# TJUMMG/OCPG

Hardware: AMD Instinct MI355X
Metric: clips/sec fwd+bwd (5x384x640, R101) (higher is better)
Workload: dtype bf16

## Files before the change

include/ocpg_hip.h:

```cpp
#ifndef OCPG_HIP_H
#define OCPG_HIP_H
#include <stdint.h>

#ifdef __cplusplus
extern "C" {
#endif

int ocpg_msda_fwd_f32(const float* value, const int64_t* shapes, const int64_t* level_start,
                      const float* loc, const float* attn,
                      int N, int S, int M, int D, int L, int Lq, int P,
                      float* out, const int64_t* shapes_host, void* stream);
int ocpg_msda_fwd_f64(const double* value, const int64_t* shapes, const int64_t* level_start,
                      const double* loc, const double* attn,
                      int N, int S, int M, int D, int L, int Lq, int P,
                      double* out, void* stream);

int ocpg_msda_bwd_f32(const float* value, const int64_t* shapes, const int64_t* level_start,
                      const float* loc, const float* attn, const float* grad_out,
                      int N, int S, int M, int D, int L, int Lq, int P,
                      float* grad_value, float* grad_loc, float* grad_attn,
                      const int64_t* shapes_host, void* stream);
int ocpg_msda_bwd_value_f32(const float* loc, const float* attn, const float* grad_out,
                            int N, int S, int M, int D, int L, int Lq, int P,
                            float* grad_value, const int64_t* shapes_host, void* stream);
// ... 31 lines not shown
int ocpg_msda_fwd_h16(const void* value, const int64_t* shapes, const int64_t* level_start,
                      const float* loc, const float* attn,
                      int N, int S, int M, int D, int L, int Lq, int P,
                      void* out, const int64_t* shapes_host, int dtype, void* stream);
int ocpg_msda_bwd_h16(const void* value, const int64_t* shapes, const int64_t* level_start,
                      const float* loc, const float* attn, const void* grad_out,
                      int N, int S, int M, int D, int L, int Lq, int P,
                      float* grad_value, float* grad_loc, float* grad_attn,
                      const int64_t* shapes_host, int* sel_state, int dtype, void* stream);
int ocpg_msda_bwd_value_h16(const float* loc, const float* attn, const void* grad_out,
                            int N, int S, int M, int D, int L, int Lq, int P,
                            float* grad_value, const int64_t* shapes_host, int* sel_state, int dtype, void* stream);
int ocpg_msda_bwd_locattn_h16(const void* value, const int64_t* shapes, const int64_t* level_start,
                              const float* loc, const float* attn, const void* grad_out,
                              int N, int S, int M, int D, int L, int Lq, int P,
                              float* grad_loc, float* grad_attn, int dtype, void* stream);
int ocpg_msda_fused_fwd_h16(const void* value, const int64_t* shapes, const int64_t* level_start,
                            const float* qproj, const float* ref,
                            int N, int S, int M, int D, int L, int Lq, int P,
                            void* out, float* loc_out, float* attn_out, int dtype, void* stream);
int ocpg_msda_fused_bwd_qproj_h16(const void* value, const int64_t* shapes, const int64_t* level_start,
                                  const float* loc, const float* attn, const void* grad_out,
                                  int N, int S, int M, int D, int L, int Lq, int P,
                                  float* grad_qproj, int dtype, void* stream);

int ocpg_bn_act_fwd(const void* x, const float* scale, const float* shift, const void* skip, void* y,
                    long long n_outer, int C, long long inner, int relu, int dtype, void* stream);
int ocpg_bn_act_bwd(const void* gy, const void* y, const float* scale, void* gx, void* gskip,
                    long long n_outer, int C, long long inner, int relu, int dtype, void* stream);

int ocpg_gemm_dgrad_bn_tile(long long M, int N, int K);
int ocpg_gemm_dgrad_bn(const void* a, const void* w, const void* c, const void* mask, const float* scale, void* out, void* out_skip,
                       long long M, int N, int K, int dtype, int tile, void* stream);

int ocpg_win_attn_fwd(const void* qkv, const float* biasT, const int* region, float scale, int BW, int NW, int N, int H,
                      int head_dim, void* out, float* lse, int dtype, void* stream);
int ocpg_win_attn_bwd(const void* qkv, const float* bias, const float* biasT, const int* region, float scale, int BW, int NW,
                      int N, int H, int head_dim, const void* out, const void* dout, const float* lse, void* dqkv, float* Dbuf,
                      float* dbiasT, int dtype, void* stream);

int ocpg_win_attn_bwd_mfma(const void* qkv, const float* bias, const float* biasT, const int* region, float scale, int BW, int NW, int N,
                           int H, int head_dim, const void* out, const void* dout, const float* lse, void* dqkv, float* Dbuf, void* dS,
                           int dtype, void* stream);

int ocpg_win_attn_dtable_supported(int N, int head_dim, int dtype, int T);
int ocpg_win_attn_bwd_mfma_dtable(const void* qkv, const float* bias, const float* biasT, const int* region, float scale, int BW, int NW,
                                  int N, int H, int head_dim, const void* out, const void* dout, const float* lse, void* dqkv, float* Dbuf,
                                  const int* tok_code, int code_off, int T, float* partials, float* dtable, int dtype, void* stream);

int ocpg_dynmask_fwd_f32(const float* feats, const float* params, const float* refpix, int BT, int Q, int C, int H, int W,
                         int stride, float* out, float* pre1, void* stream);

int ocpg_dynmask_bwd_pre_f32(const float* dout, const float* pre1, const float* params, int BT, int Q, int C, int H, int W,
                             int stride, float* dpre, float* part, float* w0d, void* stream);
int ocpg_dynmask_bwd_fin_f32(const float* part, const float* params, const float* refpix, const float* dw0, int BT, int Q, int C,
                             int H, int W, float* dparams, float* dref, void* stream);

int ocpg_im2col3x3_nhwc(const void* x, int N, int H, int W, int C, int stride, int dil, void* cols, int dtype, void* stream);
int ocpg_col2im3x3_nhwc(const void* dcols, int N, int H, int W, int C, int stride, int dil, void* dx, int dtype, void* stream);

int ocpg_conv3x3_mfma_fwd(const void* x, const void* w, const float* scale, const float* bias, int relu, int N, int H, int W,
                          int Cin, int Cout, int stride, void* y, void* stream);
int ocpg_conv3x3_mfma_fwd_cols(const void* x, const void* w, const float* scale, const float* bias, int relu, int N, int H, int W, int Cin,
                               int Cout, int stride, void* y, void* cols, void* stream);
int ocpg_conv3x3_mfma_dgrad(const void* dy, const void* wT, int N, int H, int W, int Cin, int Cout, int stride, void* dx,
                            void* stream);
int ocpg_conv3x3_mfma_dgrad_masked(const void* dy, const void* wT, const void* mask_y, const float* scale, int N, int H, int W, int Cin,
                                   int Cout, int stride, void* dx, void* stream);
int ocpg_conv3x3_mfma_dgrad_w(const void* dy, const void* w, const void* mask_y, const float* scale, int N, int H, int W, int Cin, int Cout,
                              int stride, void* dx, void* stream);
int ocpg_conv3x3_mfma_body_splits(long long M, int ncols, int kchannels);
int ocpg_conv3x3_mfma_fwd_bn_splitk(const void* x, const void* w, const float* scale, const float* shift, int relu, int N, int H, int W, int Cin,
                                    int Cout, int stride, int splits, float* part, void* y, void* stream);
int ocpg_conv3x3_mfma_dgrad_w_splitk(const void* dy, const void* w, const void* mask_y, const float* scale, int N, int H, int W, int Cin,
                                     int Cout, int stride, int splits, float* part, void* dx, void* stream);
int ocpg_conv3x3_mfma_wgrad_splits(int N, int H, int W, int Cin, int Cout, int stride);
int ocpg_conv3x3_mfma_wgrad(const void* gz, const void* x, int N, int H, int W, int Cin, int Cout, int stride, void* part, void* stream);
int ocpg_conv3x3_mfma_fwd_cols_h16(const void* x, const void* w, const float* scale, const float* bias, int relu, int N, int H, int W, int Cin,
                                   int Cout, int stride, void* y, void* cols, int dtype, void* stream);
int ocpg_conv3x3_mfma_dgrad_w_h16(const void* dy, const void* w, const void* mask_y, const float* scale, int N, int H, int W, int Cin, int Cout,
                                  int stride, void* dx, int dtype, void* stream);
int ocpg_conv3x3_mfma_wgrad_h16(const void* gz, const void* x, int N, int H, int W, int Cin, int Cout, int stride, void* part, int dtype,
                                void* stream);
int ocpg_conv3x3_mfma_dgrad_w_s2(const void* dy, const void* w, const void* mask_y, const float* scale, int N, int H, int W, int Cin, int Cout,
                                 int stride, void* dx, void* stream);
int ocpg_conv3x3_mfma_dgrad_w_s2_h16(const void* dy, const void* w, const void* mask_y, const float* scale, int N, int H, int W, int Cin, int Cout,
                                     int stride, void* dx, int dtype, void* stream);

int ocpg_conv3x3_mfma_splits(int N, int H, int W, int Cin, int Cout, int stride);
int ocpg_conv3x3_mfma_fwd_splitk(const void* x, const void* w, const float* bias, int N, int H, int W, int Cin, int Cout, int stride,
                                 int splits, float* part, void* y, int out_dt, void* cols, void* stream);
int ocpg_conv3x3_mfma_fwd_splitk_h16(const void* x, const void* w, const float* bias, int N, int H, int W, int Cin, int Cout, int stride,
                                     int splits, float* part, void* y, int out_dt, void* cols, int dtype, void* stream);

int ocpg_gemm(const void* A, const void* B, void* C, const void* bias, int dtype, int out_dtype, int transA, int transB,
              long long M, long long N, long long K, long long lda, long long ldb, long long ldc, long long batch,
              long long strideA, long long strideB, long long strideC, float alpha, float beta, void* stream);
long long ocpg_gemm_plans(void);
long long ocpg_gemm_tuned(long long* changed);
long long ocpg_gemm_tune_rejected(void);
void ocpg_gemm_set_tuning(int on);
long long ocpg_gemm_export_picks(long long* buf, long long cap_pairs);
int ocpg_gemm_import_picks(const long long* buf, long long n_pairs);
int ocpg_gemm_bn_act(const void* A, const void* W, void* D, const float* scale, const float* shift, const void* skip, int relu, int dtype,
                     long long M, long long N, long long K, void* stream);

int ocpg_levelset_fwd_f32(const float* x, const float* feats, const float* box, int Lr, int N, int C, int CF, int h, int w, float* sums,
                          float* coef, float* loss, void* stream);
int ocpg_levelset_bwd_f32(const float* x, const float* feats, const float* box, const float* coef, const float* gloss, int Lr, int N,
                          int C, int CF, int h, int w, float* gx, float* gfeat, void* stream);
int ocpg_proj_fwd_f32(const float* x, const float* tcmax, const float* trmax, const float* tcmean, const float* trmean, int Lr, int B,
                      int T, int H, int W, float* colstat, float* rowstat, float* IU, float* loss, void* stream);
int ocpg_proj_bwd_f32(const float* x, const float* tcmax, const float* trmax, const float* tcmean, const float* trmean,
                      const float* colstat, const float* rowstat, const float* IU, const float* gloss, int Lr, int B, int T, int H, int W,
                      float* Gc, float* Gr, float* gx, void* stream);

int ocpg_matcher_cost_f32(const float* logits, const float* boxes, const float* masks, long long sl, long long sb, long long st,
                          long long sq, const float* gt, const float* tboxes, const float* valid, const long long* labels, int Lr,
                          int B, int T, int Q, int K, int h, int w, float wc, float wb, float wg, float wm, float wd, float* sums,
                          float* cost, int* bad, void* stream);

int ocpg_dropout_add_ln_fwd(const void* x, const float* res, const float* gamma, const float* beta, long long R, int C, float eps, float p,
                            unsigned long long seed, unsigned long long offset, const unsigned long long* rng_base, int x_dtype, float* y,
                            float* mean, float* rstd, void* stream);
int ocpg_dropout_add_ln_bwd(const float* gy, const void* x, const float* res, const float* gamma, const float* mean, const float* rstd,
                            long long R, int C, float p, unsigned long long seed, unsigned long long offset, const unsigned long long* rng_base,
                            int x_dtype, void* gx, float* gres, float* dgb_part, void* stream);
long long ocpg_dropout_add_ln_bwd_slots(long long R);
int ocpg_bias_relu_dropout_fwd(const void* a, const void* bias, long long R, int C, float p, unsigned long long seed,
                               unsigned long long offset, const unsigned long long* rng_base, int dtype, void* h, void* stream);
int ocpg_bias_relu_dropout_bwd(const void* gh, const void* h, long long R, int C, float p, int dtype, void* ga, float* dbias_part,
                               void* stream);
long long ocpg_bias_relu_dropout_bwd_slots(long long R, int C, int dtype);

int ocpg_multi_cast(const long long* srcs, const long long* dsts, const long long* numels, const long long* chunk_prefix, int n,
                    long long total_chunks, int src_dtype, int dst_dtype, void* stream);
int ocpg_multi_cast_sum(const long long* srcs, const long long* dsts, const long long* numels, const long long* chunk_prefix,
                        const long long* splits, const long long* strides, int n, long long total_chunks, int src_dtype, int dst_dtype,
                        void* stream);
long long ocpg_colsum_blocks(long long R);
int ocpg_colsum_partials(const void* x, long long R, int C, int dtype, float* part, void* stream);

int ocpg_grad_norm_clip(const long long* grads, const long long* numels, const long long* chunk_prefix, int n, long long total_chunks,
                        float max_norm, float* partials, float* norm_and_coef, void* stream);
int ocpg_adamw_step(const long long* params, const long long* grads, const long long* exp_avg, const long long* exp_avg_sq,
                    const long long* numels, const long long* chunk_prefix, const float* lr, const float* weight_decay, int n,
                    long long total_chunks, const float* norm_and_coef, double beta1, double beta2, double eps, long long step, void* stream);
int ocpg_grad_norm_clip_amp(const long long* grads, const long long* numels, const long long* chunk_prefix, int n, long long total_chunks,
                            float max_norm, float* partials, const float* grad_scale, const float* found_inf, double beta1, double beta2,
                            float* amp_state, void* stream);
int ocpg_adamw_step_amp(const long long* params, const long long* grads, const long long* exp_avg, const long long* exp_avg_sq,
                        const long long* numels, const long long* chunk_prefix, const float* lr, const float* weight_decay, int n,
                        long long total_chunks, const float* amp_state, double beta1, double beta2, double eps, void* stream);

int ocpg_det_loss_fwd_f32(const float* logits, const float* boxes, const long long* src, const float* valid, const long long* labels,
                          const float* tboxes, const float* num_boxes, float alpha, int Lr, int B, int T, int Q, int K, float* loss, int* bad,
                          void* stream);
int ocpg_det_loss_bwd_f32(const float* logits, const float* boxes, const long long* src, const float* valid, const long long* labels,
                          const float* tboxes, const float* num_boxes, const float* gloss, float alpha, int Lr, int B, int T, int Q, int K,
                          float* glogits, float* gboxes, void* stream);

int ocpg_spectral_gate_fwd(const void* X, const float* coef, const float* high, int N, int C, int hw, float* out, void* stream);
int ocpg_spectral_c2p(const void* X, const float* coef, const float* high, int N, int C, int hw, void* pair, int dtype, void* stream);
int ocpg_spectral_p2c(const void* pair, const void* Xs, const float* coef, const float* high, int N, int C, int hw, void* out, float* part,
                      int dtype, void* stream);
int ocpg_spectral_gate_bwd(const float* gout, const void* X, const float* coef, const float* high, int N, int C, int hw, void* dX, float* part,
// ... 81 lines not shown
```

ocpg_amd/_lib.py:

```python
import ctypes
import os

import torch

_HERE = os.path.dirname(os.path.abspath(__file__))
LIB_PATH = os.environ.get("OCPG_HIP_LIB") or os.path.join(_HERE, "lib", "libocpg_hip.so")
_lib = None

_i64p = ctypes.c_void_p
_vp = ctypes.c_void_p
_int = ctypes.c_int

SIGNATURES = {
    "ocpg_msda_fwd_f32": [_vp, _i64p, _i64p, _vp, _vp] + [_int] * 7 + [_vp, _vp, _vp],
    "ocpg_msda_fwd_f64": [_vp, _i64p, _i64p, _vp, _vp] + [_int] * 7 + [_vp, _vp],
    "ocpg_msda_bwd_f32": [_vp, _i64p, _i64p, _vp, _vp, _vp] + [_int] * 7 + [_vp, _vp, _vp, _vp, _vp],
    "ocpg_msda_bwd_value_f32": [_vp, _vp, _vp] + [_int] * 7 + [_vp, _vp, _vp],
    "ocpg_msda_fused_fwd_f32": [_vp, _i64p, _i64p, _vp, _vp] + [_int] * 7 + [_vp, _vp, _vp, _vp],
    "ocpg_msda_fused_bwd_qproj_f32": [_vp, _i64p, _i64p, _vp, _vp, _vp] + [_int] * 7 + [_vp, _vp],
    "ocpg_msda_bwd_value_sel_f32": [_vp, _vp, _vp] + [_int] * 7 + [_vp, _vp, _vp, _vp],
    "ocpg_msda_bwd_locattn_f32": [_vp, _i64p, _i64p, _vp, _vp, _vp] + [_int] * 7 + [_vp, _vp, _vp],
    "ocpg_msda_bwd_f64": [_vp, _i64p, _i64p, _vp, _vp, _vp] + [_int] * 7 + [_vp, _vp, _vp, _vp],
    "ocpg_msda_sf_fwd_f32": [_vp, _vp, _vp, _vp, _i64p, _i64p, _vp, _vp] + [_int] * 7 + [_vp, _vp, _vp, _vp],
    "ocpg_msda_sf_bwd_f32": [_vp, _vp, _vp, _vp, _i64p, _i64p, _vp, _vp, _vp] + [_int] * 7 + [_vp, _vp, _vp, _vp],
    "ocpg_msda_sf_bwd_params_f32": [_vp, _vp, _vp] + [_int] * 4 + [_vp, _vp, _vp],
    "ocpg_msda_fwd_h16": [_vp, _i64p, _i64p, _vp, _vp] + [_int] * 7 + [_vp, _vp, _int, _vp],
    "ocpg_msda_bwd_h16": [_vp, _i64p, _i64p, _vp, _vp, _vp] + [_int] * 7 + [_vp, _vp, _vp, _vp, _vp, _int, _vp],
    "ocpg_msda_bwd_value_h16": [_vp, _vp, _vp] + [_int] * 7 + [_vp, _vp, _vp, _int, _vp],
    "ocpg_msda_bwd_locattn_h16": [_vp, _i64p, _i64p, _vp, _vp, _vp] + [_int] * 7 + [_vp, _vp, _int, _vp],
    "ocpg_msda_fused_fwd_h16": [_vp, _i64p, _i64p, _vp, _vp] + [_int] * 7 + [_vp, _vp, _vp, _int, _vp],
    "ocpg_msda_fused_bwd_qproj_h16": [_vp, _i64p, _i64p, _vp, _vp, _vp] + [_int] * 7 + [_vp, _int, _vp],
    "ocpg_bn_act_fwd": [_vp, _vp, _vp, _vp, _vp, ctypes.c_longlong, _int, ctypes.c_longlong, _int, _int, _vp],
    "ocpg_bn_act_bwd": [_vp, _vp, _vp, _vp, _vp, ctypes.c_longlong, _int, ctypes.c_longlong, _int, _int, _vp],
    "ocpg_gemm_dgrad_bn_tile": [ctypes.c_longlong, _int, _int],
    "ocpg_gemm_dgrad_bn": [_vp] * 7 + [ctypes.c_longlong, _int, _int, _int, _int, _vp],
    "ocpg_dynmask_fwd_f32": [_vp, _vp, _vp] + [_int] * 6 + [_vp, _vp, _vp],
    "ocpg_dynmask_bwd_pre_f32": [_vp, _vp, _vp] + [_int] * 6 + [_vp, _vp, _vp, _vp],
    "ocpg_dynmask_bwd_fin_f32": [_vp, _vp, _vp, _vp] + [_int] * 5 + [_vp, _vp, _vp],
    "ocpg_conv3x3_mfma_fwd": [_vp, _vp, _vp, _vp] + [_int] * 7 + [_vp, _vp],
    "ocpg_conv3x3_mfma_fwd_cols": [_vp, _vp, _vp, _vp] + [_int] * 7 + [_vp, _vp, _vp],
    "ocpg_conv3x3_mfma_dgrad": [_vp, _vp] + [_int] * 6 + [_vp, _vp],
    "ocpg_conv3x3_mfma_dgrad_masked": [_vp, _vp, _vp, _vp] + [_int] * 6 + [_vp, _vp],
    "ocpg_conv3x3_mfma_dgrad_w": [_vp, _vp, _vp, _vp] + [_int] * 6 + [_vp, _vp],
    "ocpg_conv3x3_mfma_splits": [_int] * 6,
    "ocpg_conv3x3_mfma_wgrad_splits": [_int] * 6,
    "ocpg_conv3x3_mfma_body_splits": [ctypes.c_longlong, _int, _int],
    "ocpg_conv3x3_mfma_fwd_bn_splitk": [_vp, _vp, _vp, _vp] + [_int] * 8 + [_vp, _vp, _vp],
    "ocpg_conv3x3_mfma_dgrad_w_splitk": [_vp, _vp, _vp, _vp] + [_int] * 7 + [_vp, _vp, _vp],
    "ocpg_conv3x3_mfma_wgrad": [_vp, _vp] + [_int] * 6 + [_vp, _vp],
    "ocpg_conv3x3_mfma_fwd_cols_h16": [_vp, _vp, _vp, _vp] + [_int] * 7 + [_vp, _vp, _int, _vp],
    "ocpg_conv3x3_mfma_dgrad_w_h16": [_vp, _vp, _vp, _vp] + [_int] * 6 + [_vp, _int, _vp],
    "ocpg_conv3x3_mfma_wgrad_h16": [_vp, _vp] + [_int] * 6 + [_vp, _int, _vp],
    "ocpg_conv3x3_mfma_dgrad_w_s2": [_vp, _vp, _vp, _vp] + [_int] * 6 + [_vp, _vp],
    "ocpg_conv3x3_mfma_dgrad_w_s2_h16": [_vp, _vp, _vp, _vp] + [_int] * 6 + [_vp, _int, _vp],
    "ocpg_conv3x3_mfma_fwd_splitk": [_vp, _vp, _vp] + [_int] * 7 + [_vp, _vp, _int, _vp, _vp],
    "ocpg_conv3x3_mfma_fwd_splitk_h16": [_vp, _vp, _vp] + [_int] * 7 + [_vp, _vp, _int, _vp, _int, _vp],
    "ocpg_gemm": [_vp, _vp, _vp, _vp] + [_int] * 4 + [ctypes.c_longlong] * 10 + [ctypes.c_float, ctypes.c_float, _vp],
    "ocpg_gemm_plans": [],
    "ocpg_gemm_tuned": [_vp],
    "ocpg_gemm_tune_rejected": [],
    "ocpg_gemm_set_tuning": [_int],
    "ocpg_gemm_export_picks": [_vp, ctypes.c_longlong],
    "ocpg_gemm_import_picks": [_vp, ctypes.c_longlong],
    "ocpg_window_means3x3_fwd": [_vp, ctypes.c_longlong, _int, _int, _int, _vp, _vp],
    "ocpg_window_means3x3_bwd": [_vp, ctypes.c_longlong, _int, _int, _vp, _vp],
    "ocpg_window_sums3x3_cl_bands": [_int],
    "ocpg_window_sums3x3_cl": [_vp, _int, _int, _int, _int, _int, _vp, _vp],
    "ocpg_window_means3x3_bwd_cl": [_vp, _int, _int, _int, _int, _vp, _vp, _vp],
    "ocpg_mso_conv3x3": [_vp, _int, _int, _vp, _int, _vp, _vp, _int, _vp, _int, _vp, _vp, _int] + [_int] * 6 + [_vp],
    "ocpg_mso_wgrad_rows": [_int] * 4,
    "ocpg_mso_wgrad": [_vp, _int, _int, _vp, _vp, _vp] + [_int] * 8 + [_vp],
    "ocpg_bilinear_nhwc_fwd": [_vp] + [_int] * 6 + [_vp, _vp],
    "ocpg_bilinear_nhwc_bwd": [_vp] + [_int] * 6 + [_vp, _vp],
    "ocpg_small_linear_fwd": [_vp, _int, _vp, _vp, _int, _int, _int, _int, _vp, _vp],
    "ocpg_small_linear_bwd": [_vp, _int, _vp, _int, _vp, _vp, _int, _int, _int, _vp, _vp, _vp, _vp],
    "ocpg_small_linear_fwd_h16": [_vp, _int, _vp, _vp, _int, _int, _int, _int, _vp, _int, _vp],
    "ocpg_small_linear_bwd_h16": [_vp, _int, _vp, _int, _vp, _vp, _int, _int, _int, _vp, _vp, _vp, _int, _vp],
    "ocpg_small_linear_f32_fwd": [_vp, _vp, _vp, _int, _int, _int, _vp, _vp],
    "ocpg_small_linear_f32_bwd": [_vp, _vp, _vp, _int, _int, _int, _vp, _vp, _vp, _vp],
    "ocpg_layernorm_blocks": [ctypes.c_longlong],
    "ocpg_groupnorm_cl_work": [ctypes.c_longlong, _int, _int, _int],
    "ocpg_groupnorm_cl_fwd": [_vp, _int, _vp, _vp, ctypes.c_longlong, _int, _int, _int, ctypes.c_float, _vp, _vp, _vp, _vp, _vp],
    "ocpg_groupnorm_cl_bwd": [_vp, _vp, _int, _vp, _vp, _vp, ctypes.c_longlong, _int, _int, _int, _vp, _vp, _vp, _vp],
    "ocpg_groupnorm_cl2cl_fwd": [_vp, _int, _vp, _vp, ctypes.c_longlong, _int, _int, _int, ctypes.c_float, _vp, _vp, _vp, _vp, _vp],
    "ocpg_groupnorm_cl2cl_bwd": [_vp, _vp, _int, _vp, _vp, _vp, ctypes.c_longlong, _int, _int, _int, _vp, _vp, _vp, _vp],
    "ocpg_layernorm_fwd": [_vp, _int, _vp, _vp, ctypes.c_longlong, _int, ctypes.c_float, _vp, _int, _vp, _vp, _vp],
    "ocpg_layernorm_bwd": [_vp, _int, _vp, _int, _vp, _vp, _vp, ctypes.c_longlong, _int, _vp, _int, _vp, _vp, _vp],
    "ocpg_gather_rows_bwd": [_vp, _vp, _vp, _int, _int, _vp, _vp],
    "ocpg_relpos_bias_fwd": [_vp, _vp, _int, ctypes.c_longlong, _int, _vp, _vp, _vp],
    "ocpg_relpos_bias_bwd": [_vp, _vp, _vp, _int, _int, _int, _int, _vp, _vp],
    "ocpg_gather_rows_pad": [_vp, _vp] + [ctypes.c_longlong] * 4 + [_vp, _vp],
    "ocpg_graph_replace_memsets": [_vp, _vp],
    "ocpg_graph_stats": [_vp, _vp],
    "ocpg_graph_memcpy_nodes": [_vp, _vp, _int],
    "ocpg_gemm_bn_act": [_vp] * 6 + [_int, _int] + [ctypes.c_longlong] * 3 + [_vp],
    "ocpg_levelset_fwd_f32": [_vp] * 3 + [_int] * 6 + [_vp] * 4,
    "ocpg_levelset_bwd_f32": [_vp] * 5 + [_int] * 6 + [_vp] * 3,
    "ocpg_proj_fwd_f32": [_vp] * 5 + [_int] * 5 + [_vp] * 5,
    "ocpg_proj_bwd_f32": [_vp] * 9 + [_int] * 5 + [_vp] * 4,
    "ocpg_matcher_cost_f32": [_vp] * 3 + [ctypes.c_longlong] * 4 + [_vp] * 4 + [_int] * 7 + [ctypes.c_float] * 5 + [_vp] * 4,
    "ocpg_dropout_add_ln_fwd": [_vp] * 4 + [ctypes.c_longlong, _int, ctypes.c_float, ctypes.c_float, ctypes.c_ulonglong, ctypes.c_ulonglong, _vp, _int]
                               + [_vp] * 4,
    "ocpg_dropout_add_ln_bwd": [_vp] * 6 + [ctypes.c_longlong, _int, ctypes.c_float, ctypes.c_ulonglong, ctypes.c_ulonglong, _vp, _int] + [_vp] * 4,
    "ocpg_dropout_add_ln_bwd_slots": [ctypes.c_longlong],
    "ocpg_bias_relu_dropout_fwd": [_vp, _vp, ctypes.c_longlong, _int, ctypes.c_float, ctypes.c_ulonglong, ctypes.c_ulonglong, _vp, _int, _vp, _vp],
    "ocpg_bias_relu_dropout_bwd": [_vp, _vp, ctypes.c_longlong, _int, ctypes.c_float, _int, _vp, _vp, _vp],
    "ocpg_bias_relu_dropout_bwd_slots": [ctypes.c_longlong, _int, _int],
    "ocpg_multi_cast": [_vp] * 4 + [_int, ctypes.c_longlong, _int, _int, _vp],
    "ocpg_multi_cast_sum": [_vp] * 6 + [_int, ctypes.c_longlong, _int, _int, _vp],
    "ocpg_colsum_blocks": [ctypes.c_longlong],
    "ocpg_grad_norm_clip": [_vp] * 3 + [_int, ctypes.c_longlong, ctypes.c_float, _vp, _vp, _vp],
    "ocpg_adamw_step": [_vp] * 8 + [_int, ctypes.c_longlong, _vp, ctypes.c_double, ctypes.c_double, ctypes.c_double, ctypes.c_longlong, _vp],
    "ocpg_grad_norm_clip_amp": [_vp] * 3 + [_int, ctypes.c_longlong, ctypes.c_float, _vp, _vp, _vp, ctypes.c_double, ctypes.c_double, _vp, _vp],
    "ocpg_adamw_step_amp": [_vp] * 8 + [_int, ctypes.c_longlong, _vp, ctypes.c_double, ctypes.c_double, ctypes.c_double, _vp],
    "ocpg_lfm_dft_supported": [_int, _int],
    "ocpg_lfm_dft_split": [_int],
    "ocpg_lfm_spectrum_fwd": [_vp, _vp, _vp] + [_int] * 4 + [_vp, _vp, ctypes.c_float, _vp, _vp, _int, _vp],
    "ocpg_lfm_spectrum_inv": [_vp, _int, _vp, _vp, _vp, _vp] + [_int] * 4 + [_vp, _vp, ctypes.c_float, _vp, _vp, _vp, _vp],
    "ocpg_colsum_partials": [_vp, ctypes.c_longlong, _int, _int, _vp, _vp],
    "ocpg_det_loss_fwd_f32": [_vp] * 7 + [ctypes.c_float] + [_int] * 5 + [_vp] * 3,
    "ocpg_det_loss_bwd_f32": [_vp] * 8 + [ctypes.c_float] + [_int] * 5 + [_vp] * 3,
    "ocpg_spectral_gate_fwd": [_vp] * 3 + [_int] * 3 + [_vp, _vp],
    "ocpg_spectral_gate_bwd": [_vp] * 4 + [_int] * 3 + [_vp, _vp, _vp],
    "ocpg_spectral_c2p": [_vp] * 3 + [_int] * 3 + [_vp, _int, _vp],
    "ocpg_spectral_p2c": [_vp] * 4 + [_int] * 3 + [_vp, _vp, _int, _vp],
    "ocpg_masked_ce_fwd_f32": [_vp] * 3 + [_int, ctypes.c_longlong, _vp, _vp],
    "ocpg_masked_ce_bwd_f32": [_vp] * 4 + [_int, ctypes.c_longlong, _vp, _vp],
    "ocpg_im2col3x3_nhwc": [_vp] + [_int] * 6 + [_vp, _int, _vp],
    "ocpg_col2im3x3_nhwc": [_vp] + [_int] * 6 + [_vp, _int, _vp],
    "ocpg_attn_smallk_fwd": [_vp, ctypes.c_longlong, _vp, ctypes.c_longlong, _vp, ctypes.c_longlong, _vp, ctypes.c_float] + [_int] * 5
                            + [ctypes.c_float, ctypes.c_ulonglong, ctypes.c_ulonglong, _vp, _vp, ctypes.c_longlong, _vp, _int, _vp],
    "ocpg_attn_smallk_bwd": [_vp, ctypes.c_longlong, _vp, ctypes.c_longlong, _vp, ctypes.c_longlong, _vp, _vp, ctypes.c_longlong, _vp,
                             ctypes.c_float] + [_int] * 5 + [ctypes.c_float, ctypes.c_ulonglong, ctypes.c_ulonglong, _vp, _vp, ctypes.c_longlong,
                                                             _vp, _vp, _int, _vp],
    "ocpg_win_attn_fwd": [_vp, _vp, _vp, ctypes.c_float] + [_int] * 5 + [_vp, _vp, _int, _vp],
    "ocpg_win_attn_bwd": [_vp, _vp, _vp, _vp, ctypes.c_float] + [_int] * 5 + [_vp] * 6 + [_int, _vp],
    "ocpg_win_attn_bwd_mfma": [_vp, _vp, _vp, _vp, ctypes.c_float] + [_int] * 5 + [_vp] * 6 + [_int, _vp],
    "ocpg_win_attn_dtable_supported": [_int] * 4,
    "ocpg_win_attn_bwd_mfma_dtable": [_vp, _vp, _vp, _vp, ctypes.c_float] + [_int] * 5 + [_vp] * 6 + [_int, _int, _vp, _vp, _int, _vp],
}


_TIMING = {"on": False, "events": []}
_UNTIMED = ("ocpg_win_attn_dtable_supported", "ocpg_conv3x3_mfma_body_splits", "ocpg_gemm_dgrad_bn_tile", "ocpg_conv3x3_mfma_wgrad_splits", "ocpg_window_sums3x3_cl_bands", "ocpg_lfm_dft_supported", "ocpg_lfm_dft_split", "ocpg_conv3x3_mfma_splits", "ocpg_gemm_set_tuning", "ocpg_gemm_export_picks", "ocpg_gemm_import_picks", "ocpg_colsum_blocks", "ocpg_mso_wgrad_rows", "ocpg_gemm_plans", "ocpg_gemm_tuned", "ocpg_gemm_tune_rejected", "ocpg_bias_relu_dropout_bwd_slots", "ocpg_dropout_add_ln_bwd_slots", "ocpg_groupnorm_cl_work")


def enable_kernel_timing(on=True):
    _TIMING["on"] = on
    _TIMING["events"] = []


def collect_kernel_timing(work=None):
    torch.cuda.synchronize()
    out = {}
    for name, args, e0, e1 in _TIMING["events"]:
        d = out.setdefault(name, {"ms": 0.0, "n": 0, "work": 0.0, "modelled": 0})
        d["ms"] += e0.elapsed_time(e1)
        d["n"] += 1
        w = work(name, args) if work is not None else None
        if isinstance(w, tuple):
            d["work_lowp"] = d.get("work_lowp", 0.0) + (w[0] if w[1] else 0.0)
            w = w[0]
        if w is not None:
            d["work"] += w
            d["modelled"] += 1
    _TIMING["events"] = []
    _TIMING["on"] = False
    return out


CENSUS = {"on": False, "calls": {}}
CENSUS_ALSO = {"ocpg_conv3x3_mfma_dgrad_w_s2": "ocpg_conv3x3_mfma_dgrad_w", "ocpg_conv3x3_mfma_dgrad_w_s2_h16": "ocpg_conv3x3_mfma_dgrad_w_h16"}


def census(on=True):
    CENSUS["on"] = on
    if on:
        CENSUS["calls"] = {}
    return CENSUS["calls"]


class _Lib:

    def __init__(self, cdll):
        self._cdll = cdll

    def __getattr__(self, name):
        fn = getattr(self._cdll, name)
        if name not in SIGNATURES or name in _UNTIMED:
            setattr(self, name, fn)
            return fn
        timed = not name.startswith("ocpg_msda_")

        def call(*a):
            if CENSUS["on"]:
                rc = fn(*a)
                if rc == 0:
                    for k in (name, CENSUS_ALSO.get(name)):
                        if k is not None:
                            CENSUS["calls"][k] = CENSUS["calls"].get(k, 0) + 1
                return rc
            if not (timed and _TIMING["on"]):
                return fn(*a)
            e0, e1 = torch.cuda.Event(enable_timing=True), torch.cuda.Event(enable_timing=True)
            e0.record()
            rc = fn(*a)
            e1.record()
            _TIMING["events"].append((name, tuple(getattr(x, "value", x) for x in a), e0, e1))
            return rc
        setattr(self, name, call)
        return call


def lib():
    global _lib
    if _lib is None:
        if not os.path.exists(LIB_PATH):
            raise RuntimeError(
                f"{LIB_PATH} not found: build it with `python -m ocpg_amd.csrc.build` "
                "(hipcc --offload-arch=gfx950). The HIP extension is mandatory; there is no CPU/PyTorch fallback.")
        L = ctypes.CDLL(LIB_PATH)
        for name, argtypes in SIGNATURES.items():
            fn = getattr(L, name)
            fn.argtypes = argtypes
            fn.restype = ctypes.c_int
        L.ocpg_hip_version.restype = ctypes.c_char_p
        L.ocpg_gemm_plans.restype = ctypes.c_longlong
# ... 29 lines not shown
```

ocpg_amd/csrc/conv3x3_wgrad.hip:

```cpp
#include <hip/hip_bf16.h>
#include <hip/hip_fp16.h>
#include <hip/hip_runtime.h>
#include <stdint.h>

#include <cstdlib>

#include "../../include/ocpg_hip.h"
#include "h16_elem.h"

namespace {

typedef ocpg_h16::h16x8 bf16x8;
typedef short s4 __attribute__((ext_vector_type(4)));
typedef ocpg_h16::f32x16 f32x16;
using ocpg_h16::Bf16;
using ocpg_h16::Fp16;

constexpr int NT = 256, TM = 64, TN = 64, LROW = 72;

__device__ __forceinline__ bf16x8 tr_frag(const short* tile, int r0, int pitch, int c0, int lane) {
  const int li = lane & 15, grp = lane >> 4, fh = lane >> 5;
  const short* p = tile + (r0 + (8 * fh + (li >> 2)) * pitch) * LROW + c0 + 16 * (grp & 1) + 4 * (li & 3);
  const s4 lo = __builtin_amdgcn_ds_read_tr16_b64_v4i16((__attribute__((address_space(3))) s4*)p);
  const s4 hi = __builtin_amdgcn_ds_read_tr16_b64_v4i16((__attribute__((address_space(3))) s4*)(p + 4 * pitch * LROW));
  bf16x8 r;
  r[0] = lo[0]; r[1] = lo[1]; r[2] = lo[2]; r[3] = lo[3]; r[4] = hi[0]; r[5] = hi[1]; r[6] = hi[2]; r[7] = hi[3];
  return r;
}

__device__ __forceinline__ uint4 keep(uint4 v, bool yes) { return make_uint4(yes ? v.x : 0u, yes ? v.y : 0u, yes ? v.z : 0u, yes ? v.w : 0u); }

struct WG {
  int N, H, W, Ho, Wo, Cin, Cout, stride, seg, xw, rows_per_split;
};

#define WGRAD_KERNEL conv3x3_wgrad
#define WGRAD_ELEM Bf16
#include "conv3x3_wgrad_kernel.h"
#undef WGRAD_KERNEL
#undef WGRAD_ELEM
#define WGRAD_KERNEL conv3x3_wgrad_f16
#define WGRAD_ELEM Fp16
#include "conv3x3_wgrad_kernel.h"
#undef WGRAD_KERNEL
#undef WGRAD_ELEM

inline int seg_of(int stride) { return stride == 1 ? 64 : 32; }

}

extern "C" {

int ocpg_conv3x3_mfma_wgrad_splits(int N, int H, int W, int Cin, int Cout, int stride) {
  if (N <= 0 || H <= 0 || W <= 0 || Cin <= 0 || Cout <= 0 || (stride != 1 && stride != 2)) return 0;
  const long long rows = (long long)N * ((H - 1) / stride + 1);
  const long long tiles = (long long)((Cout + TM - 1) / TM) * ((Cin + TN - 1) / TN);
  static const int target = [] { const char* e = std::getenv("OCPG_WGRAD_WGS"); return e && *e ? std::atoi(e) : 256; }();
  long long s = (target + tiles - 1) / tiles;
  if (s > rows) s = rows;
  if (s < 1) s = 1;
  const long long rps = (rows + s - 1) / s;
  return (int)((rows + rps - 1) / rps);
}

int ocpg_conv3x3_mfma_wgrad_h16(const void* gz, const void* x, int N, int H, int W, int Cin, int Cout, int stride, void* part, int dtype,
                                void* stream) {
  if (dtype != 1 && dtype != 2) return -1010;
  if (N < 0 || H <= 0 || W <= 0 || Cin <= 0 || Cout <= 0) return -1003;
  if ((stride != 1 && stride != 2) || Cin % 8 != 0 || Cout % 8 != 0) return -2000;
  if (N == 0) return 0;
  if (!gz) return -1001;
  if (!x) return -1002;
  if (!part) return -1009;
  WG g;
  g.N = N; g.H = H; g.W = W; g.Ho = (H - 1) / stride + 1; g.Wo = (W - 1) / stride + 1; g.Cin = Cin; g.Cout = Cout; g.stride = stride;
  g.seg = seg_of(stride);
  g.xw = (g.seg - 1) * stride + 3;
  const int splits = ocpg_conv3x3_mfma_wgrad_splits(N, H, W, Cin, Cout, stride);
  const long long rows = (long long)N * g.Ho;
  g.rows_per_split = (int)((rows + splits - 1) / splits);
  const dim3 grid((unsigned)((Cout + TM - 1) / TM), (unsigned)((Cin + TN - 1) / TN), (unsigned)splits);
  if (dtype == 2) {
    if (stride == 1) conv3x3_wgrad_f16<1, 64><<<grid, NT, 0, (hipStream_t)stream>>>((const __half*)gz, (const __half*)x, g, (__half*)part);
    else conv3x3_wgrad_f16<2, 32><<<grid, NT, 0, (hipStream_t)stream>>>((const __half*)gz, (const __half*)x, g, (__half*)part);
  } else if (stride == 1) {
    conv3x3_wgrad<1, 64><<<grid, NT, 0, (hipStream_t)stream>>>((const __hip_bfloat16*)gz, (const __hip_bfloat16*)x, g, (__hip_bfloat16*)part);
  } else {
    conv3x3_wgrad<2, 32><<<grid, NT, 0, (hipStream_t)stream>>>((const __hip_bfloat16*)gz, (const __hip_bfloat16*)x, g, (__hip_bfloat16*)part);
  }
  const hipError_t e = hipGetLastError();
  return e == hipSuccess ? 0 : -(int)e;
}

int ocpg_conv3x3_mfma_wgrad(const void* gz, const void* x, int N, int H, int W, int Cin, int Cout, int stride, void* part, void* stream) {
  return ocpg_conv3x3_mfma_wgrad_h16(gz, x, N, H, W, Cin, Cout, stride, part, 1, stream);
}

}
```

ocpg_amd/csrc/conv3x3_wgrad_kernel.h:

```cpp
template <int S, int SEG>
#ifdef WG_ONE_SET
__global__ __launch_bounds__(NT) __attribute__((amdgpu_waves_per_eu(2, 2))) void WGRAD_KERNEL(
#else
__global__ __launch_bounds__(NT) __attribute__((amdgpu_waves_per_eu(1, 1))) void WGRAD_KERNEL(
#endif
    const WGRAD_ELEM::T* __restrict__ gz, const WGRAD_ELEM::T* __restrict__ x, WG g,
                                                    WGRAD_ELEM::T* __restrict__ part) {
  using E = WGRAD_ELEM;
  using T = E::T;
  constexpr int XW = (SEG - 1) * S + 3;
  constexpr int GL = SEG * 8 / NT;
  constexpr int XL = (3 * XW * 8 + NT - 1) / NT;
  __shared__ __attribute__((aligned(16))) short Gs[SEG * LROW];
  __shared__ __attribute__((aligned(16))) short Xs[3 * XW * LROW];
  const int tid = threadIdx.x, lane = tid & 63, wave = tid >> 6, wm = wave & 1, wn = wave >> 1;
  const int co0 = blockIdx.x * TM, ci0 = blockIdx.y * TN;
  const long long rows = (long long)g.N * g.Ho;
  const long long r_lo = (long long)blockIdx.z * g.rows_per_split, r_hi = min(rows, r_lo + g.rows_per_split);
  const int nseg = (g.Wo + SEG - 1) / SEG;
  const int nchunks = (int)(r_hi > r_lo ? r_hi - r_lo : 0) * nseg;
  f32x16 acc[9];
#pragma unroll
  for (int t = 0; t < 9; ++t)
#pragma unroll
    for (int r = 0; r < 16; ++r) acc[t][r] = 0.f;
  struct Regs { uint4 rg[GL], rx[XL]; unsigned zg, zx; };
  Regs RA, RB;
  const long long r0c = min(r_lo, rows - 1);
  int fn = (int)(r0c / g.Ho), fy = (int)(r0c - (long long)fn * g.Ho), fs = 0;
  auto fetch = [&](Regs& R) __attribute__((always_inline)) {
    uint4 (&rg)[GL] = R.rg; uint4 (&rx)[XL] = R.rx;
    unsigned zg = 0, zx = 0;
    const int xo0 = fs * SEG, npx = min(SEG, g.Wo - xo0);
    const long long grow = ((long long)fn * g.Ho + fy) * g.Wo;
#pragma unroll
    for (int i = 0; i < GL; ++i) {
      const int e = tid + i * NT, k = e >> 3, sg = e & 7;
      const bool ok = k < npx && co0 + sg * 8 + 8 <= g.Cout;
      zg |= ok ? 0u : 1u << i;
      rg[i] = *reinterpret_cast<const uint4*>(gz + (grow + min(xo0 + k, g.Wo - 1)) * g.Cout + min(co0 + sg * 8, g.Cout - 8));
    }
#pragma unroll
    for (int i = 0; i < XL; ++i) {
      const int e = min(tid + i * NT, 3 * XW * 8 - 1), sg = e & 7, j = (e >> 3) % XW, ky = (e >> 3) / XW;
      const int yi = fy * S + ky - 1, xi = xo0 * S - 1 + j;
      const bool ok = yi >= 0 && yi < g.H && xi >= 0 && xi < g.W && ci0 + sg * 8 + 8 <= g.Cin;
      zx |= ok ? 0u : 1u << i;
      rx[i] = *reinterpret_cast<const uint4*>(x + (((long long)fn * g.H + min(max(yi, 0), g.H - 1)) * g.W + min(max(xi, 0), g.W - 1)) * g.Cin +
                                              min(ci0 + sg * 8, g.Cin - 8));
    }
    R.zg = zg, R.zx = zx;
    if (fs + 1 < nseg) ++fs;
    else if ((long long)fn * g.Ho + fy + 1 < r_hi) { fs = 0; if (++fy == g.Ho) { fy = 0; ++fn; } }
  };
  auto park = [&](const Regs& R) __attribute__((always_inline)) {
    const uint4 (&rg)[GL] = R.rg; const uint4 (&rx)[XL] = R.rx;
    const unsigned zg = R.zg, zx = R.zx;
#pragma unroll
    for (int i = 0; i < GL; ++i) {
      const int e = tid + i * NT;
      *reinterpret_cast<uint4*>(Gs + (e >> 3) * LROW + (e & 7) * 8) = keep(rg[i], !((zg >> i) & 1u));
    }
#pragma unroll
    for (int i = 0; i < XL; ++i) {
      const int e = tid + i * NT;
      if (e < 3 * XW * 8) *reinterpret_cast<uint4*>(Xs + (e >> 3) * LROW + (e & 7) * 8) = keep(rx[i], !((zx >> i) & 1u));
    }
  };
  fetch(RA);
#ifndef WG_ONE_SET
  fetch(RB);
#endif
  int ps = 0;
  auto chunk = [&](Regs& R) __attribute__((always_inline)) {
    const int npx = min(SEG, g.Wo - ps * SEG), kp = (npx + 15) & ~15;
    if (++ps == nseg) ps = 0;
    __syncthreads();
#ifndef WG_CUT_LOAD
    park(R);
    __syncthreads();
    fetch(R);
#endif
#ifndef WG_CUT_COMPUTE
    for (int k0 = 0; k0 < kp; k0 += 16) {
      const bf16x8 a = tr_frag(Gs, k0, 1, wm * 32, lane);
#pragma unroll
      for (int t = 0; t < 9; ++t) {
        const int ky = t / 3, kx = t - ky * 3;
        const bf16x8 b = tr_frag(Xs + ky * XW * LROW, k0 * S + kx, S, wn * 32, lane);
        acc[t] = E::mfma(a, b, acc[t]);
      }
    }
#endif
  };
#ifdef WG_ONE_SET
  for (int c = 0; c < nchunks; ++c) chunk(RA);
#else
  for (int c = 0; c < nchunks; c += 2) {
    chunk(RA);
    if (c + 1 < nchunks) chunk(RB);
  }
#endif
  const int ci = ci0 + wn * 32 + (lane & 31);
  if (ci < g.Cin) {
    T* out = part + (long long)blockIdx.z * g.Cout * 9 * g.Cin;
#pragma unroll
    for (int t = 0; t < 9; ++t)
#pragma unroll
      for (int r = 0; r < 16; ++r) {
        const int co = co0 + wm * 32 + (r & 3) + 8 * (r >> 2) + 4 * (lane >> 5);
        if (co < g.Cout) out[((long long)co * 9 + t) * g.Cin + ci] = E::narrow(acc[t][r]);
      }
  }
}
```

Before: 61.91.

## Add pipelined double-buffered conv3x3 wgrad kernel with XCD-aware block remap

Adds a PIPE variant of the 3x3 weight-gradient MFMA kernel, enabled by default. It double-buffers the LDS tiles so the next chunk is stored while the current one is multiplied, keeps three register sets of prefetched global loads in flight, and software-pipelines LDS fragment loads against MFMAs. It also remaps block indices across 8 XCDs and stages the output through LDS for vectorized 16-byte stores. The cost is double the LDS footprint and more registers, which may lower occupancy, and it can be turned off with an env var or a setter.

```diff
diff --git a/include/ocpg_hip.h b/include/ocpg_hip.h
--- a/include/ocpg_hip.h
+++ b/include/ocpg_hip.h
@@ -137,6 +137,7 @@
                                   int stride, void* dx, int dtype, void* stream);
 int ocpg_conv3x3_mfma_wgrad_h16(const void* gz, const void* x, int N, int H, int W, int Cin, int Cout, int stride, void* part, int dtype,
                                 void* stream);
+int ocpg_conv3x3_wgrad_set_pipelined(int on);
 int ocpg_conv3x3_mfma_dgrad_w_s2(const void* dy, const void* w, const void* mask_y, const float* scale, int N, int H, int W, int Cin, int Cout,
                                  int stride, void* dx, void* stream);
 int ocpg_conv3x3_mfma_dgrad_w_s2_h16(const void* dy, const void* w, const void* mask_y, const float* scale, int N, int H, int W, int Cin, int Cout,
diff --git a/ocpg_amd/_lib.py b/ocpg_amd/_lib.py
--- a/ocpg_amd/_lib.py
+++ b/ocpg_amd/_lib.py
@@ -51,6 +51,7 @@
     "ocpg_conv3x3_mfma_fwd_cols_h16": [_vp, _vp, _vp, _vp] + [_int] * 7 + [_vp, _vp, _int, _vp],
     "ocpg_conv3x3_mfma_dgrad_w_h16": [_vp, _vp, _vp, _vp] + [_int] * 6 + [_vp, _int, _vp],
     "ocpg_conv3x3_mfma_wgrad_h16": [_vp, _vp] + [_int] * 6 + [_vp, _int, _vp],
+    "ocpg_conv3x3_wgrad_set_pipelined": [_int],
     "ocpg_conv3x3_mfma_dgrad_w_s2": [_vp, _vp, _vp, _vp] + [_int] * 6 + [_vp, _vp],
     "ocpg_conv3x3_mfma_dgrad_w_s2_h16": [_vp, _vp, _vp, _vp] + [_int] * 6 + [_vp, _int, _vp],
     "ocpg_conv3x3_mfma_fwd_splitk": [_vp, _vp, _vp] + [_int] * 7 + [_vp, _vp, _int, _vp, _vp],
@@ -142,7 +143,7 @@
 
 
 _TIMING = {"on": False, "events": []}
-_UNTIMED = ("ocpg_win_attn_dtable_supported", "ocpg_conv3x3_mfma_body_splits", "ocpg_gemm_dgrad_bn_tile", "ocpg_conv3x3_mfma_wgrad_splits", "ocpg_window_sums3x3_cl_bands", "ocpg_lfm_dft_supported", "ocpg_lfm_dft_split", "ocpg_conv3x3_mfma_splits", "ocpg_gemm_set_tuning", "ocpg_gemm_export_picks", "ocpg_gemm_import_picks", "ocpg_colsum_blocks", "ocpg_mso_wgrad_rows", "ocpg_gemm_plans", "ocpg_gemm_tuned", "ocpg_gemm_tune_rejected", "ocpg_bias_relu_dropout_bwd_slots", "ocpg_dropout_add_ln_bwd_slots", "ocpg_groupnorm_cl_work")
+_UNTIMED = ("ocpg_win_attn_dtable_supported", "ocpg_conv3x3_wgrad_set_pipelined", "ocpg_conv3x3_mfma_body_splits", "ocpg_gemm_dgrad_bn_tile", "ocpg_conv3x3_mfma_wgrad_splits", "ocpg_window_sums3x3_cl_bands", "ocpg_lfm_dft_supported", "ocpg_lfm_dft_split", "ocpg_conv3x3_mfma_splits", "ocpg_gemm_set_tuning", "ocpg_gemm_export_picks", "ocpg_gemm_import_picks", "ocpg_colsum_blocks", "ocpg_mso_wgrad_rows", "ocpg_gemm_plans", "ocpg_gemm_tuned", "ocpg_gemm_tune_rejected", "ocpg_bias_relu_dropout_bwd_slots", "ocpg_dropout_add_ln_bwd_slots", "ocpg_groupnorm_cl_work")
 
 
 def enable_kernel_timing(on=True):
diff --git a/ocpg_amd/csrc/conv3x3_wgrad.hip b/ocpg_amd/csrc/conv3x3_wgrad.hip
--- a/ocpg_amd/csrc/conv3x3_wgrad.hip
+++ b/ocpg_amd/csrc/conv3x3_wgrad.hip
@@ -3,6 +3,7 @@
 #include <hip/hip_runtime.h>
 #include <stdint.h>
 
+#include <atomic>
 #include <cstdlib>
 
 #include "../../include/ocpg_hip.h"
@@ -33,6 +34,15 @@
 struct WG {
   int N, H, W, Ho, Wo, Cin, Cout, stride, seg, xw, rows_per_split;
 };
+
+std::atomic<int> g_pipelined{-1};
+
+inline bool pipelined() {
+  const int v = g_pipelined.load(std::memory_order_relaxed);
+  if (v >= 0) return v != 0;
+  const char* e = std::getenv("OCPG_WGRAD_PIPE");
+  return !(e && e[0] == '0' && !e[1]);
+}
 
 #define WGRAD_KERNEL conv3x3_wgrad
 #define WGRAD_ELEM Bf16
@@ -80,14 +90,22 @@
   const long long rows = (long long)N * g.Ho;
   g.rows_per_split = (int)((rows + splits - 1) / splits);
   const dim3 grid((unsigned)((Cout + TM - 1) / TM), (unsigned)((Cin + TN - 1) / TN), (unsigned)splits);
+  const hipStream_t st = (hipStream_t)stream;
+  const bool pipe = pipelined() && (long long)W * Cin < (1ll << 31) && (long long)g.Wo * Cout < (1ll << 31) && ((uintptr_t)part & 15) == 0;
+#define WGRAD_LAUNCH(KERNEL, T, S, SEG)                                                                                  \
+  do {                                                                                                                   \
+    if (pipe) KERNEL<S, SEG, true><<<grid, NT, 0, st>>>((const T*)gz, (const T*)x, g, (T*)part);                        \
+    else KERNEL<S, SEG, false><<<grid, NT, 0, st>>>((const T*)gz, (const T*)x, g, (T*)part);                            \
+  } while (0)
   if (dtype == 2) {
-    if (stride == 1) conv3x3_wgrad_f16<1, 64><<<grid, NT, 0, (hipStream_t)stream>>>((const __half*)gz, (const __half*)x, g, (__half*)part);
-    else conv3x3_wgrad_f16<2, 32><<<grid, NT, 0, (hipStream_t)stream>>>((const __half*)gz, (const __half*)x, g, (__half*)part);
+    if (stride == 1) WGRAD_LAUNCH(conv3x3_wgrad_f16, __half, 1, 64);
+    else WGRAD_LAUNCH(conv3x3_wgrad_f16, __half, 2, 32);
   } else if (stride == 1) {
-    conv3x3_wgrad<1, 64><<<grid, NT, 0, (hipStream_t)stream>>>((const __hip_bfloat16*)gz, (const __hip_bfloat16*)x, g, (__hip_bfloat16*)part);
+    WGRAD_LAUNCH(conv3x3_wgrad, __hip_bfloat16, 1, 64);
   } else {
-    conv3x3_wgrad<2, 32><<<grid, NT, 0, (hipStream_t)stream>>>((const __hip_bfloat16*)gz, (const __hip_bfloat16*)x, g, (__hip_bfloat16*)part);
+    WGRAD_LAUNCH(conv3x3_wgrad, __hip_bfloat16, 2, 32);
   }
+#undef WGRAD_LAUNCH
   const hipError_t e = hipGetLastError();
   return e == hipSuccess ? 0 : -(int)e;
 }
@@ -96,4 +114,6 @@
   return ocpg_conv3x3_mfma_wgrad_h16(gz, x, N, H, W, Cin, Cout, stride, part, 1, stream);
 }
 
+int ocpg_conv3x3_wgrad_set_pipelined(int on) { return g_pipelined.exchange(on == 0 || on == 1 ? on : -1, std::memory_order_relaxed); }
+
 }
diff --git a/ocpg_amd/csrc/conv3x3_wgrad_kernel.h b/ocpg_amd/csrc/conv3x3_wgrad_kernel.h
--- a/ocpg_amd/csrc/conv3x3_wgrad_kernel.h
+++ b/ocpg_amd/csrc/conv3x3_wgrad_kernel.h
@@ -1,4 +1,4 @@
-template <int S, int SEG>
+template <int S, int SEG, bool PIPE>
 #ifdef WG_ONE_SET
 __global__ __launch_bounds__(NT) __attribute__((amdgpu_waves_per_eu(2, 2))) void WGRAD_KERNEL(
 #else
@@ -11,12 +11,22 @@
   constexpr int XW = (SEG - 1) * S + 3;
   constexpr int GL = SEG * 8 / NT;
   constexpr int XL = (3 * XW * 8 + NT - 1) / NT;
-  __shared__ __attribute__((aligned(16))) short Gs[SEG * LROW];
-  __shared__ __attribute__((aligned(16))) short Xs[3 * XW * LROW];
+  constexpr int GSZ = SEG * LROW, XSZ = 3 * XW * LROW;
+  __shared__ __attribute__((aligned(16))) short Gs[(PIPE ? 2 : 1) * GSZ];
+  __shared__ __attribute__((aligned(16))) short Xs[(PIPE ? 2 : 1) * XSZ];
   const int tid = threadIdx.x, lane = tid & 63, wave = tid >> 6, wm = wave & 1, wn = wave >> 1;
-  const int co0 = blockIdx.x * TM, ci0 = blockIdx.y * TN;
+  unsigned bx = blockIdx.x, by = blockIdx.y, bz = blockIdx.z;
+  if constexpr (PIPE) {
+    constexpr unsigned XCDS = 8;
+    const unsigned total = gridDim.x * gridDim.y * gridDim.z;
+    if (total % XCDS == 0) {
+      const unsigned lin = bx + gridDim.x * (by + gridDim.y * bz), v = lin % XCDS * (total / XCDS) + lin / XCDS;
+      bx = v % gridDim.x, by = v / gridDim.x % gridDim.y, bz = v / (gridDim.x * gridDim.y);
+    }
+  }
+  const int co0 = bx * TM, ci0 = by * TN;
   const long long rows = (long long)g.N * g.Ho;
-  const long long r_lo = (long long)blockIdx.z * g.rows_per_split, r_hi = min(rows, r_lo + g.rows_per_split);
+  const long long r_lo = (long long)bz * g.rows_per_split, r_hi = min(rows, r_lo + g.rows_per_split);
   const int nseg = (g.Wo + SEG - 1) / SEG;
   const int nchunks = (int)(r_hi > r_lo ? r_hi - r_lo : 0) * nseg;
   f32x16 acc[9];
@@ -53,7 +63,7 @@
     if (fs + 1 < nseg) ++fs;
     else if ((long long)fn * g.Ho + fy + 1 < r_hi) { fs = 0; if (++fy == g.Ho) { fy = 0; ++fn; } }
   };
-  auto park = [&](const Regs& R) __attribute__((always_inline)) {
+  auto park = [&](const Regs& R, short* Gs, short* Xs) __attribute__((always_inline)) {
     const uint4 (&rg)[GL] = R.rg; const uint4 (&rx)[XL] = R.rx;
     const unsigned zg = R.zg, zx = R.zx;
 #pragma unroll
@@ -67,43 +77,179 @@
       if (e < 3 * XW * 8) *reinterpret_cast<uint4*>(Xs + (e >> 3) * LROW + (e & 7) * 8) = keep(rx[i], !((zx >> i) & 1u));
     }
   };
-  fetch(RA);
+  if constexpr (PIPE) {
+    constexpr int XH = XW * 8 / NT, LEFT = XW * 8 - XH * NT, XN = 3 * XH + 1;
+    static_assert(XH * 32 + (LEFT + 7) / 8 == XW && LEFT > 0 && LEFT % 8 == 0 && 3 * LEFT <= NT && GL * 32 == SEG, "slot layout");
+    struct Set { uint4 rg[GL], rx[XN]; unsigned z; };
+    Set RA, RB, RC;
+    const int pj = tid >> 3, sg8 = (tid & 7) * 8;
+    const bool gch = co0 + sg8 + 8 <= g.Cout, xch = ci0 + sg8 + 8 <= g.Cin;
+    const unsigned gco = min(co0 + sg8, g.Cout - 8), xco = min(ci0 + sg8, g.Cin - 8);
+    const int q = min(tid, 3 * LEFT - 1), qky = q / LEFT, qj = XH * 32 + (q % LEFT >> 3), qs8 = (q & 7) * 8;
+    const bool qch = ci0 + qs8 + 8 <= g.Cin;
+    const unsigned qco = min(ci0 + qs8, g.Cin - 8);
+    auto fetch = [&](Set& R) __attribute__((always_inline)) {
+      const int xo0 = fs * SEG, npx = min(SEG, g.Wo - xo0), xb = xo0 * S - 1;
+      const char* grow = reinterpret_cast<const char*>(gz + ((long long)fn * g.Ho + fy) * g.Wo * g.Cout);
+      unsigned z = 0;
+#pragma unroll
+      for (int i = 0; i < GL; ++i) {
+        const int k = pj + 32 * i;
+        z |= k < npx && gch ? 0u : 1u << i;
+        R.rg[i] = *reinterpret_cast<const uint4*>(grow + ((unsigned)min(xo0 + k, g.Wo - 1) * (unsigned)g.Cout + gco) * 2u);
+      }
+      const char* xr[3];
+      bool rok[3];
+#pragma unroll
+      for (int ky = 0; ky < 3; ++ky) {
+        const int yi = fy * S + ky - 1;
+        rok[ky] = yi >= 0 && yi < g.H;
+        xr[ky] = reinterpret_cast<const char*>(x + ((long long)fn * g.H + min(max(yi, 0), g.H - 1)) * g.W * g.Cin);
+      }
+#pragma unroll
+      for (int h = 0; h < XH; ++h) {
+        const int xi = xb + pj + 32 * h;
+        const bool cok = xi >= 0 && xi < g.W && xch;
+        const unsigned off = ((unsigned)min(max(xi, 0), g.W - 1) * (unsigned)g.Cin + xco) * 2u;
+#pragma unroll
+        for (int ky = 0; ky < 3; ++ky) {
+          z |= cok && rok[ky] ? 0u : 1u << (4 + ky * XH + h);
+          R.rx[ky * XH + h] = *reinterpret_cast<const uint4*>(xr[ky] + off);
+        }
+      }
+      {
+        const int xi = xb + qj;
+        const bool ok = xi >= 0 && xi < g.W && qch && (qky == 0 ? rok[0] : qky == 1 ? rok[1] : rok[2]);
+        const char* xq = qky == 0 ? xr[0] : qky == 1 ? xr[1] : xr[2];
+        z |= ok ? 0u : 1u << (4 + 3 * XH);
+        R.rx[3 * XH] = *reinterpret_cast<const uint4*>(xq + ((unsigned)min(max(xi, 0), g.W - 1) * (unsigned)g.Cin + qco) * 2u);
+      }
+      R.z = z;
+      if (fs + 1 < nseg) ++fs;
+      else if ((long long)fn * g.Ho + fy + 1 < r_hi) { fs = 0; if (++fy == g.Ho) { fy = 0; ++fn; } }
+    };
+    auto park = [&](const Set& R, short* G, short* X) __attribute__((always_inline)) {
+      const unsigned z = R.z;
+      short* gp = G + pj * LROW + sg8;
+      short* xp = X + pj * LROW + sg8;
+#pragma unroll
+      for (int i = 0; i < GL; ++i) *reinterpret_cast<uint4*>(gp + 32 * i * LROW) = keep(R.rg[i], !((z >> i) & 1u));
+#pragma unroll
+      for (int ky = 0; ky < 3; ++ky)
+#pragma unroll
+        for (int h = 0; h < XH; ++h)
+          *reinterpret_cast<uint4*>(xp + (ky * XW + 32 * h) * LROW) = keep(R.rx[ky * XH + h], !((z >> (4 + ky * XH + h)) & 1u));
+      if (tid < 3 * LEFT) *reinterpret_cast<uint4*>(X + (qky * XW + qj) * LROW + qs8) = keep(R.rx[3 * XH], !((z >> (4 + 3 * XH)) & 1u));
+    };
+    fetch(RA); fetch(RB); fetch(RC);
+    int cs = 0, buf = 0;
+    auto mult = [&](const short* G, const short* X, int nk) __attribute__((always_inline)) {
+      bf16x8 a, an, b[9];
+      auto frag_b = [&](int k0, int t) __attribute__((always_inline)) {
+        const int ky = t / 3, kx = t - ky * 3;
+        return tr_frag(X + ky * XW * LROW, k0 * S + kx, S, wn * 32, lane);
+      };
+      a = tr_frag(G, 0, 1, wm * 32, lane);
+#pragma unroll
+      for (int t = 0; t < 9; ++t) b[t] = frag_b(0, t);
+      for (int k0 = 0; k0 < nk * 16; k0 += 16) {
+        const int k1 = min(k0 + 16, SEG - 16);
+#pragma unroll
+        for (int t = 0; t < 9; ++t) {
+          acc[t] = E::mfma(a, b[t], acc[t]);
+          b[t] = frag_b(k1, t);
+          if (t == 1) an = tr_frag(G, k1, 1, wm * 32, lane);
+          __builtin_amdgcn_sched_barrier(0);
+        }
+        a = an;
+      }
+    };
+    auto step = [&](Set& R, int c) __attribute__((always_inline)) {
+      const int npx = min(SEG, g.Wo - cs * SEG), nk = (npx + 15) >> 4;
+      if (++cs == nseg) cs = 0;
+      const short* G = Gs + buf * GSZ;
+      const short* X = Xs + buf * XSZ;
+      if (c < nchunks) mult(G, X, nk);
+      buf ^= 1;
+      if (c + 1 < nchunks) park(R, Gs + buf * GSZ, Xs + buf * XSZ);
+      fetch(R);
+      __syncthreads();
+    };
+    if (nchunks > 0) {
+      park(RA, Gs, Xs);
+      fetch(RA);
+      __syncthreads();
+      int c = 0;
+      do {
+        step(RB, c);
+        step(RC, c + 1);
+        step(RA, c + 2);
+        c += 3;
+      } while (c < nchunks);
+    }
+    {
+      T* out = part + (long long)bz * g.Cout * 9 * g.Cin;
+      short* stage = Xs;
+      static_assert(3 * TM * LROW <= 2 * XSZ, "staging tile");
+#pragma unroll
+      for (int t0 = 0; t0 < 9; t0 += 3) {
+        if (t0) __syncthreads();
+#pragma unroll
+        for (int t = 0; t < 3; ++t)
+#pragma unroll
+          for (int r = 0; r < 16; ++r) {
+            const T v = E::narrow(acc[t0 + t][r]);
+            stage[(t * TM + wm * 32 + (r & 3) + 8 * (r >> 2) + 4 * (lane >> 5)) * LROW + wn * 32 + (lane & 31)] = *reinterpret_cast<const short*>(&v);
+          }
+        __syncthreads();
+#pragma unroll
+        for (int i = 0; i < 3 * TM * 8 / NT; ++i) {
+          const int p = tid + i * NT, row = p >> 3, t = row / TM, co = co0 + row % TM, ci = ci0 + (p & 7) * 8;
+          if (co < g.Cout && ci + 8 <= g.Cin)
+            *reinterpret_cast<uint4*>(out + ((long long)co * 9 + t0 + t) * g.Cin + ci) = *reinterpret_cast<const uint4*>(stage + row * LROW + (p & 7) * 8);
+        }
+      }
+    }
+    return;
+  } else {
+    fetch(RA);
 #ifndef WG_ONE_SET
-  fetch(RB);
-#endif
-  int ps = 0;
-  auto chunk = [&](Regs& R) __attribute__((always_inline)) {
-    const int npx = min(SEG, g.Wo - ps * SEG), kp = (npx + 15) & ~15;
-    if (++ps == nseg) ps = 0;
-    __syncthreads();
+    fetch(RB);
+#endif
+    int ps = 0;
+    auto chunk = [&](Regs& R) __attribute__((always_inline)) {
+      const int npx = min(SEG, g.Wo - ps * SEG), kp = (npx + 15) & ~15;
+      if (++ps == nseg) ps = 0;
+      __syncthreads();
 #ifndef WG_CUT_LOAD
-    park(R);
-    __syncthreads();
-    fetch(R);
+      park(R, Gs, Xs);
+      __syncthreads();
+      fetch(R);
 #endif
 #ifndef WG_CUT_COMPUTE
-    for (int k0 = 0; k0 < kp; k0 += 16) {
-      const bf16x8 a = tr_frag(Gs, k0, 1, wm * 32, lane);
-#pragma unroll
-      for (int t = 0; t < 9; ++t) {
-        const int ky = t / 3, kx = t - ky * 3;
-        const bf16x8 b = tr_frag(Xs + ky * XW * LROW, k0 * S + kx, S, wn * 32, lane);
-        acc[t] = E::mfma(a, b, acc[t]);
-      }
-    }
-#endif
-  };
+      for (int k0 = 0; k0 < kp; k0 += 16) {
+        const bf16x8 a = tr_frag(Gs, k0, 1, wm * 32, lane);
+#pragma unroll
+        for (int t = 0; t < 9; ++t) {
+          const int ky = t / 3, kx = t - ky * 3;
+          const bf16x8 b = tr_frag(Xs + ky * XW * LROW, k0 * S + kx, S, wn * 32, lane);
+          acc[t] = E::mfma(a, b, acc[t]);
+        }
+      }
+#endif
+    };
 #ifdef WG_ONE_SET
-  for (int c = 0; c < nchunks; ++c) chunk(RA);
+    for (int c = 0; c < nchunks; ++c) chunk(RA);
 #else
-  for (int c = 0; c < nchunks; c += 2) {
-    chunk(RA);
-    if (c + 1 < nchunks) chunk(RB);
+    for (int c = 0; c < nchunks; c += 2) {
+      chunk(RA);
+      if (c + 1 < nchunks) chunk(RB);
+    }
+#endif
   }
-#endif
   const int ci = ci0 + wn * 32 + (lane & 31);
   if (ci < g.Cin) {
-    T* out = part + (long long)blockIdx.z * g.Cout * 9 * g.Cin;
+    T* out = part + (long long)bz * g.Cout * 9 * g.Cin;
 #pragma unroll
     for (int t = 0; t < 9; ++t)
 #pragma unroll
```

Result: no change. 62.32 (median of 6 runs) (+0.7%).
